# Tcadart/pyLatticeDSO

Measured on AMD Instinct MI355X. Metric: beams/s assembly+PCG-solve, higher is better.
Workload: dtype f64

## Files before the change

include/pylattice_hip.h:

```cpp
#ifndef PYLATTICE_HIP_H
#define PYLATTICE_HIP_H

#include <stdint.h>

#ifdef __cplusplus
extern "C" {
#endif

typedef struct pl_context *pl_handle;

typedef enum {
  PL_OK = 0,
  PL_ERR_ARG = -1,
  PL_ERR_HIP = -2,
  PL_ERR_STATE = -3,
  PL_ERR_NOCONV = -4,
  PL_ERR_NAN = -5,
  PL_ERR_NODEVICE = -6
} pl_status;

typedef struct {
  int64_t n_nodes;
  int64_t n_beams;
  const double *node_xyz;
// ... 185 lines not shown
                     const int32_t *beam_conn , int32_t nb,
                     const int32_t *boundary_nodes ,
                     const double *node_xyz , const double *beam_radius ,
                     const double *seg_len , const int32_t *seg_nsub ,
                     const double *u_b ,
                     const double *lam_b ,
                     double *u_full ,
                     double *lam_full ,
                     double *sens ,
                     int32_t *info );

int pl_get_records(pl_handle h, double *rec);

int pl_debug_partition(pl_handle h, int32_t *tile_of_node, int32_t *agg_of_node, int32_t *local_agg_of_node,
                       uint8_t *eliminated);

int pl_time_kernel(pl_handle h, int which, int reps, double *avg_ms);
int pl_algorithmic_bytes(pl_handle h, double *out3);
int pl_node_words_info(pl_handle h, int *classes_on, int *n_classes, int *bytes_on, int *byte_exp);
int pl_forget_history(pl_handle h);

int pl_debug_spd_solve(int device, int32_t n, const double *A, const double *b, double *x, double *quad,
                       int32_t fp32_factor);

int pl_dist_unique_id_bytes(void);
int pl_dist_unique_id(void *id_out);
int pl_dist_loopback_id(void *id_out);
int pl_dist_abort(pl_handle h);
int pl_dist_init(pl_handle h, int rank, int world, const void *unique_id, const int32_t *shared_local,
                 const int32_t *shared_global, int32_t n_shared, int32_t n_shared_global);

typedef struct pl_lattice pl_lattice;
typedef struct {
  int64_t n_nodes, n_beams, n_cell_beam, n_cell_node, n_created;
} pl_lattice_info_t;
int pl_generate_lattice(int64_t n_cells, const double *cell_coord, const double *cell_size, const double *cell_radii,
                        int32_t n_geom, int32_t n_tmpl, const double *tmpl, const int32_t *tmpl_type,
                        pl_lattice **out, pl_lattice_info_t *info);
int pl_lattice_fetch(const pl_lattice *L, double *node_xyz, int32_t *beam_conn, double *beam_radius, int32_t *beam_type,
                     int32_t *beam_cell0, int64_t *cell_beam_ptr , int64_t *cell_beam_idx,
                     int64_t *cell_node_ptr , int64_t *cell_node_idx, int32_t *created_nodes,
                     int32_t *created_beam);
void pl_lattice_free(pl_lattice *L);

int pl_penalize(int64_t n_beams, const double *node_xyz, const int32_t *beam_conn, const double *lzone ,
                double mesh_size, double *seg_len , int32_t *seg_nsub , double *pen_xyz );
// ... 16 lines not shown
```

pylatticedso_amd/_capi.py:

```python
from __future__ import annotations

import ctypes as C
import os

import numpy as np

from .timing import timing as _timing

_HERE = os.path.dirname(os.path.abspath(__file__))
LIB_PATH = os.environ.get("PYLATTICE_HIP_LIB") or os.path.join(_HERE, "libpylattice_hip.so")

PL_OK, PL_ERR_ARG, PL_ERR_HIP, PL_ERR_STATE, PL_ERR_NOCONV, PL_ERR_NAN, PL_ERR_NODEVICE = 0, -1, -2, -3, -4, -5, -6

EXPORTS = ["pl_default_opts", "pl_opts_size", "pl_stats_size", "pl_abi_version", "pl_last_error", "pl_version", "pl_lzone", "pl_create", "pl_create_ddm",
           "pl_ddm_set_preconditioner", "pl_ddm_set_geometry", "pl_ddm_update_matrices", "pl_destroy", "pl_set_bc", "pl_set_periodic",
           "pl_update_radii", "pl_set_multiplicity", "pl_update_segments", "pl_assemble", "pl_assemble_bsr", "pl_get_bsr", "pl_spmv",
           "pl_spmv_free", "pl_spmv_bsr", "pl_solve", "pl_reactions", "pl_sens", "pl_sens_gram", "pl_energy", "pl_node_mod", "pl_schur",
           "pl_stress", "pl_stress_pnorm", "pl_buckling", "pl_buckling_pnorm",
           "pl_spmv_multi", "pl_solve_multi", "pl_schur_block", "pl_geom_spmv_multi", "pl_buckling_modes", "pl_buckling_modes_sens",
           "pl_set_mass", "pl_mass_spmv_multi", "pl_vibration_modes", "pl_vibration_modes_sens",
           "pl_dyn_spmv_multi", "pl_transient",
           "pl_schur_cells", "pl_cells_recover", "pl_get_records", "pl_debug_partition", "pl_time_kernel", "pl_algorithmic_bytes", "pl_node_words_info", "pl_forget_history", "pl_debug_spd_solve", "pl_dist_unique_id_bytes",
           "pl_dist_unique_id", "pl_dist_loopback_id", "pl_dist_abort", "pl_dist_init", "pl_dist_set_peers", "pl_generate_lattice", "pl_lattice_fetch",
           "pl_lattice_free", "pl_penalize", "pl_boundary_index", "pl_boundary_index_rows"]


class PlMesh(C.Structure):
    _fields_ = [("n_nodes", C.c_int64), ("n_beams", C.c_int64), ("node_xyz", C.c_void_p),
                ("beam_conn", C.c_void_p), ("beam_radius", C.c_void_p), ("seg_len", C.c_void_p),
                ("seg_nsub", C.c_void_p)]


class PlOpts(C.Structure):
    _fields_ = [("struct_size", C.c_uint32), ("abi_version", C.c_uint32),
                ("young", C.c_double), ("poisson", C.c_double), ("kappa", C.c_double), ("pen_coef", C.c_double),
                ("device", C.c_int32), ("spmv_kernel", C.c_int32), ("precond", C.c_int32), ("reorder", C.c_int32),
                ("check_every", C.c_int32), ("lanes_per_node", C.c_int32),
                ("tile_nodes", C.c_int32), ("coarse_max_dofs", C.c_int32), ("palette", C.c_int32),
                ("local_max_dofs", C.c_int32), ("precision", C.c_int32), ("restart_every", C.c_int32),
                ("alpha_max", C.c_double), ("grid_lo", C.c_double * 3), ("grid_hi", C.c_double * 3),
                ("grid_nodes", C.c_int64), ("mintol", C.c_double), ("compact_records", C.c_int32),
                ("condense", C.c_int32), ("chol_persistent", C.c_int32), ("cg_form", C.c_int32),
                ("tile_modes", C.c_int32), ("coarse_modes", C.c_int32), ("overlap", C.c_int32),
                ("coarse_storage", C.c_int32), ("warm_start", C.c_int32), ("short_iteration", C.c_int32)]

# ... 35 lines not shown
    lib.pl_lattice_free.restype = None
    V, I32, I64, D = C.c_void_p, C.c_int32, C.c_int64, C.c_double
    sig = {"pl_default_opts": [V, C.c_uint32], "pl_opts_size": [], "pl_stats_size": [], "pl_abi_version": [], "pl_lzone": [I32, I64, I64, V, V, V, V], "pl_create": [V, V, V], "pl_create_ddm": [I64, I64, I32, V, I32, V, V, V, V],
           "pl_ddm_set_preconditioner": [V, I32, V, V], "pl_ddm_set_geometry": [V, V], "pl_ddm_update_matrices": [V, I32, V, V], "pl_destroy": [V], "pl_set_bc": [V, V, V, V], "pl_set_periodic": [V, V],
           "pl_update_radii": [V, V], "pl_set_multiplicity": [V, V], "pl_update_segments": [V, V, V], "pl_assemble": [V],
           "pl_assemble_bsr": [V, I32, V, V], "pl_get_bsr": [V, V, V, V], "pl_spmv": [V, V, V],
           "pl_spmv_free": [V, V, V], "pl_spmv_bsr": [V, V, V], "pl_solve": [V, D, I32, V, V],
           "pl_reactions": [V, V, V], "pl_sens": [V, V, V, V], "pl_sens_gram": [V, I32, V, V], "pl_energy": [V, V, V], "pl_node_mod": [V, V, V],
           "pl_stress": [V, V, I32, V, V], "pl_stress_pnorm": [V, V, I32, D, V, V, V, V],
           "pl_buckling": [V, V, I32, D, I32, V, V, V], "pl_buckling_pnorm": [V, V, I32, D, I32, D, V, V, V, V],
           "pl_schur": [V, V, I32, D, I32, V], "pl_spmv_multi": [V, I32, I32, V, V],
           "pl_solve_multi": [V, I32, V, V, D, I32, V, V], "pl_schur_block": [V, V, I32, D, I32, I32, V],
           "pl_geom_spmv_multi": [V, V, I32, I32, V, V],
           "pl_buckling_modes": [V, V, I32, I32, D, I32, D, I32, V, V, V, V, V],
           "pl_buckling_modes_sens": [V, V, I32, V, V, D, I32, V, V, V, V],
           "pl_set_mass": [V, D, I32, V], "pl_mass_spmv_multi": [V, I32, I32, V, V],
           "pl_vibration_modes": [V, I32, I32, D, I32, D, I32, V, V, V, V, V],
           "pl_vibration_modes_sens": [V, I32, V, V, V, V, V],
           "pl_dyn_spmv_multi": [V, D, D, I32, I32, V, V],
           "pl_transient": [V, I32, D, D, D, D, D, I32, V, V, V, V, D, I32, I32, V, V, V, I32, V, V, V],
           "pl_schur_cells": [V, I32, I32, I32, V, I32, V, V, V, V, V, V, V],
           "pl_cells_recover": [V, I32, I32, I32, V, I32, V, V, V, V, V, V, V, V, V, V, V],
           "pl_get_records": [V, V], "pl_debug_partition": [V, V, V, V, V], "pl_time_kernel": [V, I32, I32, V],
           "pl_algorithmic_bytes": [V, V], "pl_node_words_info": [V, V, V, V, V], "pl_forget_history": [V], "pl_debug_spd_solve": [I32, I32, V, V, V, V, I32], "pl_dist_unique_id_bytes": [], "pl_dist_unique_id": [V], "pl_dist_loopback_id": [V], "pl_dist_abort": [V],
           "pl_dist_init": [V, I32, I32, V, V, V, I32, I32], "pl_dist_set_peers": [V, V],
           "pl_generate_lattice": [I64, V, V, V, I32, I32, V, V, V, V], "pl_lattice_fetch": [V] * 12,
           "pl_lattice_free": [V], "pl_penalize": [I64, V, V, V, D, V, V, V],
           "pl_boundary_index": [I64, V, V, I64, V, V, V, V, V, V],
           "pl_boundary_index_rows": [I64, V, V, I64, V, V, V, V, V, V]}
    for name, args in sig.items():
        getattr(lib, name).argtypes = args
    if lib.pl_opts_size() != C.sizeof(PlOpts) or lib.pl_stats_size() != C.sizeof(PlStats):
        raise ImportError(f"{p}: pl_opts_t / pl_stats_t are {lib.pl_opts_size()} / {lib.pl_stats_size()} bytes in the "
                          f"library, {C.sizeof(PlOpts)} / {C.sizeof(PlStats)} in this binding (ABI version "
                          f"{lib.pl_abi_version()}): rebuild libpylattice_hip.so")
    _lib = lib
    return lib


def default_opts(lib=None) -> "PlOpts":
    lib = lib or load_library()
    opts = PlOpts()
    _check(lib, lib.pl_default_opts(C.byref(opts), C.sizeof(PlOpts)))
    return opts


def _ptr(a):
# ... 11 lines not shown
    if rc != PL_OK and rc not in allow:
        raise PlError(rc, lib.pl_last_error().decode())
    return rc


def lzone(node_xyz, beam_conn, beam_radius, device=0):
    lib = load_library()
    xyz = _f64(np.asarray(node_xyz).reshape(-1))
    conn = np.ascontiguousarray(beam_conn, dtype=np.int32).reshape(-1)
    rad = _f64(np.asarray(beam_radius).reshape(-1), len(conn) // 2)
    out = np.empty(len(conn), np.float64)
    _check(lib, lib.pl_lzone(int(device), len(xyz) // 3, len(conn) // 2, _ptr(xyz), _ptr(conn), _ptr(rad), _ptr(out)))
    return out.reshape(-1, 2)


def debug_spd_solve(A, b, device=0, fp32_factor=False):
    lib = load_library()
    A = np.ascontiguousarray(A, np.float64)
    b = np.ascontiguousarray(b, np.float64)
    x = np.empty_like(b)
    q = C.c_double()
    _check(lib, lib.pl_debug_spd_solve(device, len(b), _ptr(A), _ptr(b), _ptr(x), C.byref(q), int(bool(fp32_factor))))
    return x, q.value


MULTI_MAX = 64
SENS_GRAM_MAX = 8

SCHUR_CELLS_MAX_BOUNDARY, SCHUR_CELLS_MAX_INTERIOR, SCHUR_CELLS_MAX_BEAMS = 32, 16, 512


def schur_cells_fits(n_nodes, n_beams, n_boundary):
    return (0 < n_boundary <= SCHUR_CELLS_MAX_BOUNDARY and n_nodes - n_boundary <= SCHUR_CELLS_MAX_INTERIOR
            and 0 < n_beams <= SCHUR_CELLS_MAX_BEAMS)


def _per_instance(name, a, tail, n_inst):
    if a.shape == tail:
        a = np.broadcast_to(a, (n_inst,) + tail)
    elif a.shape != (n_inst,) + tail:
        raise ValueError(f"{name} must have shape {tail} or {(n_inst,) + tail}, got {a.shape}")
    return np.ascontiguousarray(a)


def schur_cells(node_xyz, beam_conn, boundary_nodes, beam_radius, seg_len, seg_nsub, young, poisson, kappa=0.9,
                pen_coef=1.5, device=0, n_inst=None):
# ... 755 lines not shown
```

pylatticedso_amd/csrc/pl_api.hip:

```cpp
#include <functional>

#include "pl_solver.h"
#include "pl_condense.h"
#include "pl_multi.h"
#include "pl_stress.h"
#include "pl_buckling.h"
#include "pl_geom.h"
#include "pl_mass.h"
#include "pl_dyn.h"
#include "pl_sensgram.h"


namespace {
template <typename WT>
int debug_spd_solve_t(int device, int32_t n, const double *A, const double *b, double *x, double *quad) {
  if (n <= 0 || !A || !b || !x) return fail(PL_ERR_ARG, "pl_debug_spd_solve: bad argument");
  int ndev = 0;
  if (hipGetDeviceCount(&ndev) != hipSuccess || ndev <= 0) return fail(PL_ERR_NODEVICE, "no HIP device visible");
  PL_HIP(hipSetDevice(device));
  const int np = (n + pl::kNB - 1) / pl::kNB * pl::kNB;
  std::vector<double> Ap((size_t)np * np, 0.0), bp(np, 0.0);
  for (int i = 0; i < np; ++i) {
    if (i < n) {
      std::memcpy(&Ap[(size_t)i * np], A + (size_t)i * n, n * sizeof(double));
// ... 15 lines not shown
  PL_HIP(dt.alloc(np));
  PL_HIP(dy.alloc(np));
  PL_HIP(dq.alloc(pl::kSlots));
  PL_HIP(dinfo.alloc(2));
  PL_HIP(hipMemcpy(dA.p, Ap.data(), Ap.size() * sizeof(double), hipMemcpyHostToDevice));
  PL_HIP(hipMemcpy(db.p, bp.data(), np * sizeof(double), hipMemcpyHostToDevice));
  PL_HIP(hipMemset(dW.p, 0, Ap.size() * sizeof(WT)));
  PL_HIP(hipMemset(dq.p, 0, pl::kSlots * sizeof(double)));
  PL_HIP(hipMemset(dinfo.p, 0, 2 * sizeof(int)));
  pl::dense_factor_inverse(dA.p, dL.p, dW.p, dWt.p, dD.p, np, np, dinfo.p, 0, nullptr);
  pl::dense_apply(dW.p, dWt.p, np, np, db.p, dt.p, dy.p, dq.p, nullptr, nullptr);
  PL_HIP(hipGetLastError());
  PL_HIP(hipDeviceSynchronize());
  int info[2];
  PL_HIP(hipMemcpy(info, dinfo.p, sizeof(info), hipMemcpyDeviceToHost));
  if (info[0] != 0) return fail(PL_ERR_ARG, "pl_debug_spd_solve: matrix is not positive definite");
  std::vector<double> y(np), q(pl::kSlots);
  PL_HIP(hipMemcpy(y.data(), dy.p, np * sizeof(double), hipMemcpyDeviceToHost));
  PL_HIP(hipMemcpy(q.data(), dq.p, pl::kSlots * sizeof(double), hipMemcpyDeviceToHost));
  std::memcpy(x, y.data(), n * sizeof(double));
  if (quad) {
    *quad = 0.0;
    for (double v : q) *quad += v;
  }
  return PL_OK;
}

}

extern "C" {

const char *pl_last_error(void) { return g_err.c_str(); }
#ifndef PL_KP_HASH
#define PL_KP_HASH "unknown"
#endif
const char *pl_version(void) { return "pylattice_hip 0.2 (gfx950) kp=" PL_KP_HASH; }

uint32_t pl_opts_size(void) { return (uint32_t)sizeof(pl_opts_t); }
uint32_t pl_stats_size(void) { return (uint32_t)sizeof(pl_stats_t); }
uint32_t pl_abi_version(void) { return PL_ABI_VERSION; }

int pl_default_opts(pl_opts_t *o, uint32_t struct_size) {
  if (!o) return fail(PL_ERR_ARG, "pl_default_opts: null argument");
  if (struct_size != sizeof(pl_opts_t))
    return fail(PL_ERR_ARG, "pl_default_opts: the caller's pl_opts_t has " + std::to_string(struct_size) +
                                " bytes, this library's " + std::to_string(sizeof(pl_opts_t)) +
// ... 2873 lines not shown
  PL_HIP(hipEventElapsedTime(&ms, h->ev0, h->ev1));
  *avg_ms = (double)ms / reps;
  return PL_OK;
}

int pl_node_words_info(pl_handle h, int *classes_on, int *n_classes, int *bytes_on, int *byte_exp) {
  if (!valid(h)) return fail(PL_ERR_ARG, "pl_node_words_info: null handle");
  const pl::Coarse &cs = h->coarse;
  const bool words = node_words_apply(h);
  const bool cls = words && h->assembled && cs.dcl_ready;
  const bool bytes = words && cs.rel_e >= 0;
  if (classes_on) *classes_on = cls ? 1 : 0;
  if (n_classes) *n_classes = h->assembled ? cs.dcl_classes : 0;
  if (bytes_on) *bytes_on = bytes ? 1 : 0;
  if (byte_exp) *byte_exp = bytes ? cs.rel_e : -1;
  return PL_OK;
}

int pl_debug_spd_solve(int device, int32_t n, const double *A, const double *b, double *x, double *quad,
                       int32_t fp32_factor) {
  return fp32_factor ? debug_spd_solve_t<float>(device, n, A, b, x, quad)
                     : debug_spd_solve_t<double>(device, n, A, b, x, quad);
}

int pl_lzone(int device, int64_t n_nodes, int64_t n_beams, const double *node_xyz, const int32_t *beam_conn,
             const double *beam_radius, double *lzone) {
  if (n_nodes <= 0 || n_beams <= 0 || !node_xyz || !beam_conn || !beam_radius || !lzone)
    return fail(PL_ERR_ARG, "pl_lzone: bad argument");
  int ndev = 0;
  if (hipGetDeviceCount(&ndev) != hipSuccess || ndev <= 0)
    return fail(PL_ERR_NODEVICE, "pl_lzone: no HIP device visible (libpylattice_hip has no CPU fallback)");
  if (device < 0 || device >= ndev) return fail(PL_ERR_ARG, "pl_lzone: bad device ordinal");
  const int64_t nh = 2 * n_beams;
  std::vector<int64_t> ptr((size_t)n_nodes + 1, 0);
  for (int64_t h = 0; h < nh; ++h) {
    const int32_t v = beam_conn[h];
    if (v < 0 || v >= n_nodes) return fail(PL_ERR_ARG, "pl_lzone: node id out of range");
    ptr[(size_t)v + 1]++;
  }
  for (int64_t i = 0; i < n_nodes; ++i) ptr[i + 1] += ptr[i];
  std::vector<int32_t> half((size_t)nh);
  {
    std::vector<int64_t> fill(ptr.begin(), ptr.end() - 1);
    for (int64_t h = 0; h < nh; ++h) half[(size_t)fill[beam_conn[h]]++] = (int32_t)h;
  }
  PL_HIP(hipSetDevice(device));
// ... 117 lines not shown
```

pylatticedso_amd/csrc/pl_dense.h:

```cpp
#pragma once
#include <hip/hip_runtime.h>

#include <functional>

#include <algorithm>

#include "pl_kernels.h"

namespace pl {

constexpr int kNB = 64;
constexpr int kLdT = kNB + 2;

__device__ __forceinline__ void tile_fma(const double *At, const double *Bt, int tx, int ty, double acc[4][4]) {
#pragma unroll 8
  for (int k = 0; k < kNB; ++k) {
    double a[4], b[4];
#pragma unroll
    for (int q = 0; q < 4; ++q) {
      a[q] = At[k * kLdT + 4 * ty + q];
      b[q] = Bt[k * kLdT + 4 * tx + q];
    }
#pragma unroll
    for (int i = 0; i < 4; ++i)
#pragma unroll
      for (int j = 0; j < 4; ++j) acc[i][j] += a[i] * b[j];
  }
}

__device__ __forceinline__ void stage_rows_as_k_minor(const double *G, int ld, double *T) {
  for (int e = threadIdx.x; e < kNB * kNB; e += kBlock) {
    const int row = e / kNB, k = e % kNB;
    T[k * kLdT + row] = G[(size_t)row * ld + k];
  }
}
__device__ __forceinline__ void stage_rows_as_k_major(const double *G, int ld, double *T) {
  for (int e = threadIdx.x; e < kNB * kNB; e += kBlock) {
    const int k = e / kNB, col = e % kNB;
    T[k * kLdT + col] = G[(size_t)k * ld + col];
  }
}

__device__ __forceinline__ void tile_fetch(const double *__restrict__ G, int ld, double regs[kNB * kNB / kBlock]) {
#pragma unroll
  for (int q = 0; q < kNB * kNB / kBlock; ++q) {
    const int e = threadIdx.x + q * kBlock;
    regs[q] = G[(size_t)(e / kNB) * ld + e % kNB];
  }
}
__device__ __forceinline__ void tile_store_k_minor(const double regs[kNB * kNB / kBlock], double *T) {
#pragma unroll
  for (int q = 0; q < kNB * kNB / kBlock; ++q) {
    const int e = threadIdx.x + q * kBlock;
    T[(e % kNB) * kLdT + e / kNB] = regs[q];
  }
}

constexpr int kLdD = kNB + 1;
constexpr int kHalf = kNB / 2;

constexpr int kDiagLds = kNB * kLdD + kHalf * (kHalf + 1) + kNB * 4 + 16 + 2;

__device__ __forceinline__ void chol_diag_body(double a[4][4], double *__restrict__ Akk, int ld, int kb,
                                               double *__restrict__ Dinv, int *__restrict__ info, double *lds) {
  double *Ls = lds, *T = Ls + kNB * kLdD, *colt = T + kHalf * (kHalf + 1), *dm = colt + kNB * 4;
  int &bad_s = *reinterpret_cast<int *>(dm + 16);
  static_assert(kNB == 64 && kBlock == 256, "chol_diag_body is written for 64 x 64 blocks and 256 threads");
  const int tx = threadIdx.x & 15, ty = threadIdx.x >> 4;
  const bool act = ty >= tx;
  if (threadIdx.x == 0) bad_s = 0;
  __syncthreads();
  for (int jt = 0; jt < kNB / 4; ++jt) {
    if (tx == jt && ty == jt) {
      double l[4][4], m[4][4];
      bool ok = true;
#pragma unroll
      for (int c = 0; c < 4; ++c) {
        double d = a[c][c];
#pragma unroll
        for (int q = 0; q < c; ++q) d -= l[c][q] * l[c][q];
        ok = ok && (d > 0.0);
        const double ri = rsqrt(d > 0.0 ? d : 1.0);
        l[c][c] = (d > 0.0 ? d : 1.0) * ri;
        m[c][c] = ri;
#pragma unroll
        for (int i = c + 1; i < 4; ++i) {
          double v = a[i][c];
#pragma unroll
          for (int q = 0; q < c; ++q) v -= l[i][q] * l[c][q];
          l[i][c] = v * ri;
        }
      }
      if (!ok) bad_s = 1;
#pragma unroll
      for (int c = 0; c < 4; ++c)
#pragma unroll
        for (int i = c + 1; i < 4; ++i) {
          double v = 0.0;
#pragma unroll
          for (int q = c; q < i; ++q) v -= l[i][q] * m[q][c];
          m[i][c] = v * m[i][i];
        }
#pragma unroll
      for (int i = 0; i < 4; ++i)
#pragma unroll
        for (int c = 0; c < 4; ++c) {
          a[i][c] = c <= i ? l[i][c] : 0.0;
          dm[4 * i + c] = c <= i ? m[i][c] : 0.0;
        }
    }
    __syncthreads();
    if (tx == jt && ty > jt) {
      double mm[16];
#pragma unroll
      for (int e = 0; e < 16; ++e) mm[e] = dm[e];
      double l[4][4];
#pragma unroll
      for (int i = 0; i < 4; ++i)
#pragma unroll
        for (int c = 0; c < 4; ++c) {
          double v = 0.0;
#pragma unroll
          for (int q = 0; q <= c; ++q) v += a[i][q] * mm[4 * c + q];
          l[i][c] = v;
        }
#pragma unroll
      for (int i = 0; i < 4; ++i)
#pragma unroll
        for (int c = 0; c < 4; ++c) {
          a[i][c] = l[i][c];
          colt[(4 * ty + i) * 4 + c] = l[i][c];
        }
    }
    __syncthreads();
    if (act && tx > jt) {
      double rv[4][4], cv[4][4];
#pragma unroll
      for (int i = 0; i < 4; ++i)
#pragma unroll
        for (int q = 0; q < 4; ++q) {
          rv[i][q] = colt[(4 * ty + i) * 4 + q];
          cv[i][q] = colt[(4 * tx + i) * 4 + q];
        }
#pragma unroll
      for (int i = 0; i < 4; ++i)
#pragma unroll
        for (int c = 0; c < 4; ++c)
#pragma unroll
          for (int q = 0; q < 4; ++q) a[i][c] -= rv[i][q] * cv[c][q];
    }
  }
#pragma unroll
  for (int i = 0; i < 4; ++i)
#pragma unroll
    for (int c = 0; c < 4; ++c) {
      const int row = 4 * ty + i, cx = 4 * tx + c;
      const double v = (act && cx <= row) ? a[i][c] : 0.0;
      Ls[row * kLdD + cx] = v;
      Akk[(size_t)row * ld + cx] = v;
    }
  __syncthreads();
  if (bad_s && threadIdx.x == 0) info[0] = kb * kNB + 1;
  const int lane = threadIdx.x & 63, wv = threadIdx.x >> 6;
  if (wv < 2 && lane < kHalf) {
    const int o = kHalf * wv;
    double x[kHalf];
#pragma unroll
    for (int i = 0; i < kHalf; ++i) {
      double sacc = (lane == i) ? 1.0 : 0.0;
#pragma unroll
      for (int m = 0; m < i; ++m) sacc -= Ls[(o + i) * kLdD + o + m] * x[m];
      x[i] = sacc / Ls[(o + i) * kLdD + o + i];
    }
#pragma unroll
    for (int i = 0; i < kHalf; ++i) Ls[(o + i) * kLdD + o + lane] = x[i];
  }
  __syncthreads();
  const int r = threadIdx.x & (kHalf - 1), cg = threadIdx.x / kHalf;
  {
    double t4[4] = {0, 0, 0, 0};
#pragma unroll 8
    for (int m = 0; m < kHalf; ++m) {
      const double l = Ls[(kHalf + r) * kLdD + m];
#pragma unroll
      for (int q = 0; q < 4; ++q) t4[q] += l * Ls[m * kLdD + 4 * cg + q];
    }
#pragma unroll
    for (int q = 0; q < 4; ++q) T[r * (kHalf + 1) + 4 * cg + q] = t4[q];
  }
  __syncthreads();
  {
    double o4[4] = {0, 0, 0, 0};
#pragma unroll 8
    for (int m = 0; m < kHalf; ++m) {
      const double xv = Ls[(kHalf + r) * kLdD + kHalf + m];
#pragma unroll
      for (int q = 0; q < 4; ++q) o4[q] += xv * T[m * (kHalf + 1) + 4 * cg + q];
    }
#pragma unroll
    for (int q = 0; q < 4; ++q) Ls[(kHalf + r) * kLdD + 4 * cg + q] = -o4[q];
  }
  __syncthreads();
  double *Dk = Dinv + (size_t)kb * kNB * kNB;
  for (int e = threadIdx.x; e < kNB * kNB; e += kBlock) Dk[e] = Ls[(e / kNB) * kLdD + e % kNB];
}

__global__ __launch_bounds__(kBlock) void k_chol_diag(double *__restrict__ A, int ld, int kb,
                                                     double *__restrict__ Dinv, int *__restrict__ info) {
  __shared__ double lds[kDiagLds];
  const int tx = threadIdx.x & 15, ty = threadIdx.x >> 4;
  double *Akk = A + ((size_t)kb * kNB) * ld + (size_t)kb * kNB;
  double a[4][4];
#pragma unroll
  for (int i = 0; i < 4; ++i)
#pragma unroll
    for (int c = 0; c < 4; ++c) a[i][c] = ty >= tx ? Akk[(size_t)(4 * ty + i) * ld + 4 * tx + c] : 0.0;
  chol_diag_body(a, Akk, ld, kb, Dinv, info, lds);
}

__device__ __forceinline__ void chol_step_body(double *__restrict__ A, double *__restrict__ Lf, int ld, int kb, int ib,
                                               int jb, double *__restrict__ Dinv, int *__restrict__ info, double *S) {
  double *X = S, *Y = S + kNB * kLdT, *D = S + 2 * kNB * kLdT;
  static_assert(kDiagLds <= 2 * kNB * kLdT, "diagonal-block scratch must fit into X|Y");
  const int tx = threadIdx.x & 15, ty = threadIdx.x >> 4;
  double *Aij = A + ((size_t)ib * kNB) * ld + (size_t)jb * kNB;
  double rd[kNB * kNB / kBlock], rj[kNB * kNB / kBlock], ri[kNB * kNB / kBlock], a[4][4];
  tile_fetch(Dinv + (size_t)kb * kNB * kNB, kNB, rd);
  tile_fetch(A + ((size_t)jb * kNB) * ld + (size_t)kb * kNB, ld, rj);
  if (ib != jb) tile_fetch(A + ((size_t)ib * kNB) * ld + (size_t)kb * kNB, ld, ri);
#pragma unroll
  for (int i = 0; i < 4; ++i)
#pragma unroll
    for (int j = 0; j < 4; ++j) a[i][j] = Aij[(size_t)(4 * ty + i) * ld + 4 * tx + j];
  tile_store_k_minor(rd, D);
  tile_store_k_minor(rj, X);
  __syncthreads();
  {
    double l[4][4] = {};
    tile_fma(X, D, tx, ty, l);
#pragma unroll
    for (int i = 0; i < 4; ++i)
#pragma unroll
      for (int j = 0; j < 4; ++j) Y[(4 * tx + j) * kLdT + 4 * ty + i] = l[i][j];
    if (ib == jb) {
      double *Lg = Lf + ((size_t)ib * kNB) * ld + (size_t)kb * kNB;
#pragma unroll
      for (int i = 0; i < 4; ++i)
#pragma unroll
        for (int j = 0; j < 4; ++j) Lg[(size_t)(4 * ty + i) * ld + 4 * tx + j] = l[i][j];
    }
  }
  __syncthreads();
  const double *Li = Y;
  if (ib != jb) {
    tile_store_k_minor(ri, X);
    __syncthreads();
    double l[4][4] = {};
    tile_fma(X, D, tx, ty, l);
    __syncthreads();
#pragma unroll
    for (int i = 0; i < 4; ++i)
#pragma unroll
      for (int j = 0; j < 4; ++j) X[(4 * tx + j) * kLdT + 4 * ty + i] = l[i][j];
    __syncthreads();
    Li = X;
  }
  double acc[4][4] = {};
  tile_fma(Li, Y, tx, ty, acc);
#pragma unroll
  for (int i = 0; i < 4; ++i)
#pragma unroll
    for (int j = 0; j < 4; ++j) a[i][j] -= acc[i][j];
  if (ib == kb + 1 && jb == kb + 1) {
    __syncthreads();
#pragma unroll
    for (int i = 0; i < 4; ++i)
#pragma unroll
      for (int j = 0; j < 4; ++j)
        if (ty < tx) a[i][j] = 0.0;
    chol_diag_body(a, Aij, ld, kb + 1, Dinv, info, X);
    return;
  }
#pragma unroll
  for (int i = 0; i < 4; ++i)
#pragma unroll
    for (int j = 0; j < 4; ++j) Aij[(size_t)(4 * ty + i) * ld + 4 * tx + j] = a[i][j];
}

__global__ __launch_bounds__(kBlock) void k_chol_step(double *__restrict__ A, double *__restrict__ Lf, int ld, int kb,
                                                      double *__restrict__ Dinv, int *__restrict__ info) {
  __shared__ double S[3 * kNB * kLdT];
  const int ib = kb + 1 + blockIdx.x, jb = kb + 1 + blockIdx.y;
  if (jb > ib) return;
  chol_step_body(A, Lf, ld, kb, ib, jb, Dinv, info, S);
}

constexpr int kChainMaxGrid = 196;
__device__ __forceinline__ bool chain_barrier(unsigned *bar, unsigned target, int *info) {
  __syncthreads();
  __shared__ int ok;
  if (threadIdx.x == 0) {
    __threadfence();
    atomicAdd(bar, 1u);
    int good = 1;
    unsigned spins = 0;
    while (__hip_atomic_load(bar, __ATOMIC_RELAXED, __HIP_MEMORY_SCOPE_AGENT) < target) {
      __builtin_amdgcn_s_sleep(1);
      if (++spins > (1u << 26) || __hip_atomic_load(info, __ATOMIC_RELAXED, __HIP_MEMORY_SCOPE_AGENT) == -7) {
        atomicExch(info, -7);
// ... 90 lines not shown
      o0 += a * S[m * kCw + 2 * g];
      o1 += a * S[m * kCw + 2 * g + 1];
    }
    WT *Wik = W + ((size_t)ib * kNB + r) * ld + (size_t)kb * kNB + c0 + 2 * g;
    Wik[0] = (WT)(-o0);
    Wik[1] = (WT)(-o1);
    WT *Wtki = Wt + ((size_t)kb * kNB + c0 + 2 * g) * ld + (size_t)ib * kNB + r;
    Wtki[0] = (WT)(-o0);
    Wtki[ld] = (WT)(-o1);
    if (RING && scratch && row1 < nb && ib + bw >= row1) {
      double *sc = scratch + ((size_t)kb * kNB + c0 + 2 * g) * ld + (size_t)ib * kNB + r;
      sc[0] = -o0;
      sc[ld] = -o1;
    }
    if (RING) {
      double *slot = Ws + (ib % kRing) * kNB * kCw;
      slot[r * kCw + 2 * g] = -o0;
      slot[r * kCw + 2 * g + 1] = -o1;
    }
  }
}

constexpr int kCwM = 16;
typedef double v4f64 __attribute__((ext_vector_type(4)));
template <typename WT>
__global__ __launch_bounds__(kBlock) void k_trtri_cols_mfma(const double *__restrict__ L, int ld, int nb, int bw,
                                                            const double *__restrict__ Dinv, WT *__restrict__ W,
                                                            WT *__restrict__ Wt, int row0 = 0, int row1 = 1 << 30) {
  __shared__ double At[kNB * kLdT];
  __shared__ double Ws[kNB * kCwM], S[kNB * kCwM];
  constexpr int kSl = kNB / kCwM;
  constexpr int kWr = kNB * kCwM / kBlock;
  const int kb = blockIdx.x / kSl, c0 = (blockIdx.x % kSl) * kCwM;
  row1 = min(row1, nb);
  if (kb >= row1) return;
  const bool first = kb >= row0;
  const int lane = threadIdx.x & 63, wv = threadIdx.x >> 6;
  const int li = lane & 15, lk = lane >> 4;
  if (first)
    for (int e = threadIdx.x; e < kNB * kCwM; e += kBlock) {
      const int row = e / kCwM, c = e % kCwM;
      const double v = Dinv[(size_t)kb * kNB * kNB + (size_t)row * kNB + c0 + c];
      W[((size_t)kb * kNB + row) * ld + (size_t)kb * kNB + c0 + c] = (WT)v;
      Wt[((size_t)kb * kNB + c0 + c) * ld + (size_t)kb * kNB + row] = (WT)v;
    }
  const int ib0 = first ? kb + 1 : row0;
  auto slice_fetch = [&](int jb, WT wr[kWr]) {
// ... 249 lines not shown
```

pylatticedso_amd/csrc/pl_small.h:

```cpp
#pragma once
#include "pl_coarse.h"

namespace pl {

typedef double v4f64_small __attribute__((ext_vector_type(4)));

__device__ __forceinline__ double w_entry(const float *W, size_t i) { return (double)W[i]; }
__device__ __forceinline__ double w_entry(const bf16_t *W, size_t i) {
  return (double)__uint_as_float((unsigned)reinterpret_cast<const uint16_t *>(W)[i] << 16);
}

template <typename WT>
__global__ __launch_bounds__(256) void k_dense_explicit_inverse(int n, const WT *__restrict__ W, int ld,
                                                                float *__restrict__ Ainv) {
  const int lane = threadIdx.x & 63, i = lane & 15, kq = lane >> 4;
  const int nt = n / 32;
  const long q = (long)blockIdx.x * 4 + (threadIdx.x >> 6);
  if (q >= (long)nt * (nt + 1) / 2) return;
  int ti = (int)((sqrt(8.0 * (double)q + 1.0) - 1.0) * 0.5);
  while ((long)(ti + 1) * (ti + 2) / 2 <= q) ++ti;
  while ((long)ti * (ti + 1) / 2 > q) --ti;
  const int tj = (int)(q - (long)ti * (ti + 1) / 2);
  const int a0 = 32 * ti, b0 = 32 * tj;
  v4f64_small acc[2][2];
#pragma unroll
  for (int u = 0; u < 2; ++u)
#pragma unroll
    for (int v = 0; v < 2; ++v) acc[u][v] = v4f64_small{0.0, 0.0, 0.0, 0.0};
  for (int k0 = a0; k0 < n; k0 += 8) {
    double A[2][2], B[2][2];
#pragma unroll
    for (int h = 0; h < 2; ++h) {
      const size_t row = (size_t)(k0 + 4 * h + kq) * ld;
      A[h][0] = w_entry(W, row + a0 + i);
      A[h][1] = w_entry(W, row + a0 + 16 + i);
      B[h][0] = w_entry(W, row + b0 + i);
      B[h][1] = w_entry(W, row + b0 + 16 + i);
    }
#pragma unroll
    for (int h = 0; h < 2; ++h)
#pragma unroll
      for (int u = 0; u < 2; ++u)
#pragma unroll
        for (int v = 0; v < 2; ++v) acc[u][v] = __builtin_amdgcn_mfma_f64_16x16x4f64(A[h][u], B[h][v], acc[u][v], 0, 0, 0);
  }
#pragma unroll
  for (int u = 0; u < 2; ++u)
#pragma unroll
    for (int v = 0; v < 2; ++v)
#pragma unroll
      for (int r = 0; r < 4; ++r) {
        const int a = a0 + 16 * u + kq + 4 * r, b = b0 + 16 * v + i;
        const float val = (float)acc[u][v][r];
        if (ti != tj) {
          Ainv[(size_t)a * ld + b] = val;
          Ainv[(size_t)b * ld + a] = val;
        } else if (b <= a) {
          Ainv[(size_t)a * ld + b] = val;
          Ainv[(size_t)b * ld + a] = val;
        }
      }
}

template <int TM>
__global__ __launch_bounds__(kBlock) void k_small_z(const int32_t *__restrict__ tile_start,
                                                    const int32_t *__restrict__ agg_of_tile, const double *__restrict__ cen,
                                                    const double *__restrict__ xyz, const double *__restrict__ r,
// ... 98 lines not shown
```

Baseline: 253.0 million.

## Use f64 MFMA in dense Cholesky step and simplify diagonal block inverse

Replaces the scalar 4x4 FMA tile product in the blocked Cholesky update with f64 16x16x4 MFMA instructions. The diagonal-block inverse is now built during the per-column factor sweep instead of by a separate triangular solve and product afterwards. The explicit-inverse kernel gains software prefetching of several k-steps of W. A debug entry point for the factorization is also added. The coarse/local dense factor is likely only a small part of assembly plus PCG, so the effect on the metric may be limited, and the inverse rework risks numerical or correctness regressions.

```diff
diff --git a/include/pylattice_hip.h b/include/pylattice_hip.h
--- a/include/pylattice_hip.h
+++ b/include/pylattice_hip.h
@@ -231,6 +231,8 @@
 
 int pl_debug_spd_solve(int device, int32_t n, const double *A, const double *b, double *x, double *quad,
                        int32_t fp32_factor);
+int pl_debug_spd_factor(int device, int32_t n, const double *A, int32_t bw_blocks, int32_t trtri_rows, double *L_out,
+                        double *W_out, float *Ainv32_out, int32_t *info_out);
 
 int pl_dist_unique_id_bytes(void);
 int pl_dist_unique_id(void *id_out);
diff --git a/pylatticedso_amd/_capi.py b/pylatticedso_amd/_capi.py
--- a/pylatticedso_amd/_capi.py
+++ b/pylatticedso_amd/_capi.py
@@ -20,7 +20,7 @@
            "pl_spmv_multi", "pl_solve_multi", "pl_schur_block", "pl_geom_spmv_multi", "pl_buckling_modes", "pl_buckling_modes_sens",
            "pl_set_mass", "pl_mass_spmv_multi", "pl_vibration_modes", "pl_vibration_modes_sens",
            "pl_dyn_spmv_multi", "pl_transient",
-           "pl_schur_cells", "pl_cells_recover", "pl_get_records", "pl_debug_partition", "pl_time_kernel", "pl_algorithmic_bytes", "pl_node_words_info", "pl_forget_history", "pl_debug_spd_solve", "pl_dist_unique_id_bytes",
+           "pl_schur_cells", "pl_cells_recover", "pl_get_records", "pl_debug_partition", "pl_time_kernel", "pl_algorithmic_bytes", "pl_node_words_info", "pl_forget_history", "pl_debug_spd_solve", "pl_debug_spd_factor", "pl_dist_unique_id_bytes",
            "pl_dist_unique_id", "pl_dist_loopback_id", "pl_dist_abort", "pl_dist_init", "pl_dist_set_peers", "pl_generate_lattice", "pl_lattice_fetch",
            "pl_lattice_free", "pl_penalize", "pl_boundary_index", "pl_boundary_index_rows"]
 
@@ -102,7 +102,7 @@
            "pl_schur_cells": [V, I32, I32, I32, V, I32, V, V, V, V, V, V, V],
            "pl_cells_recover": [V, I32, I32, I32, V, I32, V, V, V, V, V, V, V, V, V, V, V],
            "pl_get_records": [V, V], "pl_debug_partition": [V, V, V, V, V], "pl_time_kernel": [V, I32, I32, V],
-           "pl_algorithmic_bytes": [V, V], "pl_node_words_info": [V, V, V, V, V], "pl_forget_history": [V], "pl_debug_spd_solve": [I32, I32, V, V, V, V, I32], "pl_dist_unique_id_bytes": [], "pl_dist_unique_id": [V], "pl_dist_loopback_id": [V], "pl_dist_abort": [V],
+           "pl_algorithmic_bytes": [V, V], "pl_node_words_info": [V, V, V, V, V], "pl_forget_history": [V], "pl_debug_spd_solve": [I32, I32, V, V, V, V, I32], "pl_debug_spd_factor": [I32, I32, V, I32, I32, V, V, V, V], "pl_dist_unique_id_bytes": [], "pl_dist_unique_id": [V], "pl_dist_loopback_id": [V], "pl_dist_abort": [V],
            "pl_dist_init": [V, I32, I32, V, V, V, I32, I32], "pl_dist_set_peers": [V, V],
            "pl_generate_lattice": [I64, V, V, V, I32, I32, V, V, V, V], "pl_lattice_fetch": [V] * 12,
            "pl_lattice_free": [V], "pl_penalize": [I64, V, V, V, D, V, V, V],
@@ -160,6 +160,20 @@
     q = C.c_double()
     _check(lib, lib.pl_debug_spd_solve(device, len(b), _ptr(A), _ptr(b), _ptr(x), C.byref(q), int(bool(fp32_factor))))
     return x, q.value
+
+
+def debug_spd_factor(A, bw_blocks=0, trtri_rows=0, explicit_inverse=False, device=0):
+    lib = load_library()
+    A = np.ascontiguousarray(A, np.float64)
+    n = A.shape[0]
+    npad = (n + 63) // 64 * 64
+    L = np.empty((npad, npad), np.float64)
+    W = np.empty((npad, npad), np.float64)
+    Ainv = np.empty((npad, npad), np.float32) if explicit_inverse else None
+    info = np.zeros(1, np.int32)
+    _check(lib, lib.pl_debug_spd_factor(device, n, _ptr(A), int(bw_blocks), int(trtri_rows), _ptr(L), _ptr(W), _ptr(Ainv),
+                                        _ptr(info)))
+    return L, W, Ainv, int(info[0])
 
 
 MULTI_MAX = 64
diff --git a/pylatticedso_amd/csrc/pl_api.hip b/pylatticedso_amd/csrc/pl_api.hip
--- a/pylatticedso_amd/csrc/pl_api.hip
+++ b/pylatticedso_amd/csrc/pl_api.hip
@@ -61,6 +61,87 @@
   if (quad) {
     *quad = 0.0;
     for (double v : q) *quad += v;
+  }
+  return PL_OK;
+}
+
+int debug_spd_factor(int device, int32_t n, const double *A, int32_t bw_blocks, int32_t trtri_rows, double *L_out,
+                     double *W_out, float *Ainv32_out, int32_t *info_out) {
+  if (n <= 0 || !A || !L_out || !W_out || !info_out || bw_blocks < 0 || trtri_rows < 0)
+    return fail(PL_ERR_ARG, "pl_debug_spd_factor: bad argument");
+  int ndev = 0;
+  if (hipGetDeviceCount(&ndev) != hipSuccess || ndev <= 0) return fail(PL_ERR_NODEVICE, "no HIP device visible");
+  PL_HIP(hipSetDevice(device));
+  const int np = (n + pl::kNB - 1) / pl::kNB * pl::kNB, nb = np / pl::kNB;
+  const size_t nn = (size_t)np * np;
+  std::vector<double> Ap(nn, 0.0), Lh(nn), Wh(nn);
+  for (int i = 0; i < np; ++i) {
+    if (i < n) std::memcpy(&Ap[(size_t)i * np], A + (size_t)i * n, n * sizeof(double));
+    else Ap[(size_t)i * np + i] = 1.0;
+  }
+  DevBuf<double> dA, dL, dD, dW, dWt;
+  DevBuf<float> dW32, dAinv;
+  DevBuf<int> dinfo;
+  PL_HIP(dA.alloc(nn));
+  PL_HIP(dL.alloc(nn));
+  PL_HIP(dW.alloc(nn));
+  PL_HIP(dWt.alloc(nn));
+  PL_HIP(dD.alloc((size_t)np * pl::kNB));
+  PL_HIP(dinfo.alloc(2));
+  PL_HIP(hipMemcpy(dA.p, Ap.data(), nn * sizeof(double), hipMemcpyHostToDevice));
+  PL_HIP(hipMemset(dL.p, 0, nn * sizeof(double)));
+  PL_HIP(hipMemset(dW.p, 0, nn * sizeof(double)));
+  PL_HIP(hipMemset(dWt.p, 0, nn * sizeof(double)));
+  PL_HIP(hipMemset(dinfo.p, 0, 2 * sizeof(int)));
+  struct Side {
+    hipStream_t s = nullptr, s2 = nullptr;
+    hipEvent_t e0 = nullptr, e1 = nullptr;
+    ~Side() {
+      if (e0) (void)hipEventDestroy(e0);
+      if (e1) (void)hipEventDestroy(e1);
+      if (s2) (void)hipStreamDestroy(s2);
+      if (s) (void)hipStreamDestroy(s);
+    }
+  } sd;
+  PL_HIP(hipStreamCreateWithFlags(&sd.s, hipStreamNonBlocking));
+  pl::TrtriPhases ph;
+  if (trtri_rows > 0) {
+    PL_HIP(hipStreamCreateWithFlags(&sd.s2, hipStreamNonBlocking));
+    PL_HIP(hipEventCreateWithFlags(&sd.e0, hipEventDisableTiming));
+    PL_HIP(hipEventCreateWithFlags(&sd.e1, hipEventDisableTiming));
+    ph.stream = sd.s2;
+    ph.ev_go = sd.e0;
+    ph.ev_done = sd.e1;
+    ph.rows = trtri_rows;
+  }
+  pl::dense_factor_inverse(dA.p, dL.p, dW.p, dWt.p, dD.p, np, np, dinfo.p, bw_blocks, sd.s, nullptr, nullptr, ph);
+  PL_HIP(hipGetLastError());
+  PL_HIP(hipStreamSynchronize(sd.s));
+  int info[2];
+  PL_HIP(hipMemcpy(info, dinfo.p, sizeof(info), hipMemcpyDeviceToHost));
+  info_out[0] = info[0];
+  PL_HIP(hipMemcpy(Ap.data(), dA.p, nn * sizeof(double), hipMemcpyDeviceToHost));
+  PL_HIP(hipMemcpy(Lh.data(), dL.p, nn * sizeof(double), hipMemcpyDeviceToHost));
+  PL_HIP(hipMemcpy(Wh.data(), dW.p, nn * sizeof(double), hipMemcpyDeviceToHost));
+  for (int kb = 0; kb < nb; ++kb)
+    for (int r = 0; r < pl::kNB; ++r)
+      std::memcpy(&Lh[((size_t)kb * pl::kNB + r) * np + (size_t)kb * pl::kNB],
+                  &Ap[((size_t)kb * pl::kNB + r) * np + (size_t)kb * pl::kNB], pl::kNB * sizeof(double));
+  std::memcpy(L_out, Lh.data(), nn * sizeof(double));
+  std::memcpy(W_out, Wh.data(), nn * sizeof(double));
+  if (Ainv32_out) {
+    std::vector<float> W32(nn);
+    for (size_t e = 0; e < nn; ++e) W32[e] = (float)Wh[e];
+    PL_HIP(dW32.alloc(nn));
+    PL_HIP(dAinv.alloc(nn));
+    PL_HIP(hipMemcpy(dW32.p, W32.data(), nn * sizeof(float), hipMemcpyHostToDevice));
+    PL_HIP(hipMemset(dAinv.p, 0, nn * sizeof(float)));
+    const long tiles = (long)(np / 32) * (np / 32 + 1) / 2;
+    hipLaunchKernelGGL(pl::k_dense_explicit_inverse<float>, dim3((unsigned)((tiles + 3) / 4)), dim3(256), 0, sd.s, np,
+                       (const float *)dW32.p, np, dAinv.p);
+    PL_HIP(hipGetLastError());
+    PL_HIP(hipStreamSynchronize(sd.s));
+    PL_HIP(hipMemcpy(Ainv32_out, dAinv.p, nn * sizeof(float), hipMemcpyDeviceToHost));
   }
   return PL_OK;
 }
@@ -2980,6 +3061,10 @@
   return fp32_factor ? debug_spd_solve_t<float>(device, n, A, b, x, quad)
                      : debug_spd_solve_t<double>(device, n, A, b, x, quad);
 }
+int pl_debug_spd_factor(int device, int32_t n, const double *A, int32_t bw_blocks, int32_t trtri_rows, double *L_out,
+                        double *W_out, float *Ainv32_out, int32_t *info_out) {
+  return debug_spd_factor(device, n, A, bw_blocks, trtri_rows, L_out, W_out, Ainv32_out, info_out);
+}
 
 int pl_lzone(int device, int64_t n_nodes, int64_t n_beams, const double *node_xyz, const int32_t *beam_conn,
              const double *beam_radius, double *lzone) {
diff --git a/pylatticedso_amd/csrc/pl_dense.h b/pylatticedso_amd/csrc/pl_dense.h
--- a/pylatticedso_amd/csrc/pl_dense.h
+++ b/pylatticedso_amd/csrc/pl_dense.h
@@ -12,19 +12,16 @@
 constexpr int kNB = 64;
 constexpr int kLdT = kNB + 2;
 
-__device__ __forceinline__ void tile_fma(const double *At, const double *Bt, int tx, int ty, double acc[4][4]) {
-#pragma unroll 8
-  for (int k = 0; k < kNB; ++k) {
-    double a[4], b[4];
-#pragma unroll
-    for (int q = 0; q < 4; ++q) {
-      a[q] = At[k * kLdT + 4 * ty + q];
-      b[q] = Bt[k * kLdT + 4 * tx + q];
-    }
-#pragma unroll
-    for (int i = 0; i < 4; ++i)
-#pragma unroll
-      for (int j = 0; j < 4; ++j) acc[i][j] += a[i] * b[j];
+typedef double v4f64 __attribute__((ext_vector_type(4)));
+__device__ __forceinline__ void tile_mfma(const double *At, const double *Bt, int wv, int li, int lk, v4f64 acc[4]) {
+#pragma unroll
+  for (int s4 = 0; s4 < kNB / 4; ++s4) {
+    const double a = At[(4 * s4 + lk) * kLdT + 16 * wv + li];
+#pragma unroll
+    for (int cb = 0; cb < 4; ++cb) {
+      const double b = Bt[(4 * s4 + lk) * kLdT + 16 * cb + li];
+      acc[cb] = __builtin_amdgcn_mfma_f64_16x16x4f64(a, b, acc[cb], 0, 0, 0);
+    }
   }
 }
 
@@ -56,18 +53,16 @@
   }
 }
 
-constexpr int kLdD = kNB + 1;
-constexpr int kHalf = kNB / 2;
-
-constexpr int kDiagLds = kNB * kLdD + kHalf * (kHalf + 1) + kNB * 4 + 16 + 2;
+constexpr int kDiagLds = 2 * kNB * 4 + 16 + 2;
 
 __device__ __forceinline__ void chol_diag_body(double a[4][4], double *__restrict__ Akk, int ld, int kb,
                                                double *__restrict__ Dinv, int *__restrict__ info, double *lds) {
-  double *Ls = lds, *T = Ls + kNB * kLdD, *colt = T + kHalf * (kHalf + 1), *dm = colt + kNB * 4;
+  double *colt = lds, *xrow = colt + kNB * 4, *dm = xrow + kNB * 4;
   int &bad_s = *reinterpret_cast<int *>(dm + 16);
   static_assert(kNB == 64 && kBlock == 256, "chol_diag_body is written for 64 x 64 blocks and 256 threads");
   const int tx = threadIdx.x & 15, ty = threadIdx.x >> 4;
   const bool act = ty >= tx;
+  double mj[4][4];
   if (threadIdx.x == 0) bad_s = 0;
   __syncthreads();
   for (int jt = 0; jt < kNB / 4; ++jt) {
@@ -79,9 +74,10 @@
         double d = a[c][c];
 #pragma unroll
         for (int q = 0; q < c; ++q) d -= l[c][q] * l[c][q];
-        ok = ok && (d > 0.0);
-        const double ri = rsqrt(d > 0.0 ? d : 1.0);
-        l[c][c] = (d > 0.0 ? d : 1.0) * ri;
+        const bool pos = d > 0.0;
+        ok = ok && pos;
+        const double ri = pos ? rsqrt(d) : 0.0;
+        l[c][c] = pos ? d * ri : 1.0;
         m[c][c] = ri;
 #pragma unroll
         for (int i = c + 1; i < 4; ++i) {
@@ -106,11 +102,13 @@
 #pragma unroll
         for (int c = 0; c < 4; ++c) {
           a[i][c] = c <= i ? l[i][c] : 0.0;
-          dm[4 * i + c] = c <= i ? m[i][c] : 0.0;
+          mj[i][c] = c <= i ? m[i][c] : 0.0;
+          dm[4 * i + c] = mj[i][c];
+          xrow[16 * jt + 4 * c + i] = mj[i][c];
         }
     }
     __syncthreads();
-    if (tx == jt && ty > jt) {
+    if (tx == jt && ty != jt) {
       double mm[16];
 #pragma unroll
       for (int e = 0; e < 16; ++e) mm[e] = dm[e];
@@ -124,23 +122,25 @@
           for (int q = 0; q <= c; ++q) v += a[i][q] * mm[4 * c + q];
           l[i][c] = v;
         }
+      double *pub = (ty > jt ? colt : xrow) + 16 * ty;
 #pragma unroll
       for (int i = 0; i < 4; ++i)
 #pragma unroll
         for (int c = 0; c < 4; ++c) {
           a[i][c] = l[i][c];
-          colt[(4 * ty + i) * 4 + c] = l[i][c];
+          pub[4 * i + c] = l[i][c];
         }
     }
     __syncthreads();
-    if (act && tx > jt) {
+    if (tx > jt && (act || ty <= jt)) {
+      const double *ps = (act ? colt : xrow) + 16 * ty, *qs = colt + 16 * tx;
       double rv[4][4], cv[4][4];
 #pragma unroll
       for (int i = 0; i < 4; ++i)
 #pragma unroll
         for (int q = 0; q < 4; ++q) {
-          rv[i][q] = colt[(4 * ty + i) * 4 + q];
-          cv[i][q] = colt[(4 * tx + i) * 4 + q];
+          rv[i][q] = ps[4 * i + q];
+          cv[i][q] = qs[4 * i + q];
         }
 #pragma unroll
       for (int i = 0; i < 4; ++i)
@@ -150,59 +150,21 @@
           for (int q = 0; q < 4; ++q) a[i][c] -= rv[i][q] * cv[c][q];
     }
   }
+  if (bad_s && threadIdx.x == 0) info[0] = kb * kNB + 1;
+  double *Dk = Dinv + (size_t)kb * kNB * kNB;
 #pragma unroll
   for (int i = 0; i < 4; ++i)
 #pragma unroll
     for (int c = 0; c < 4; ++c) {
-      const int row = 4 * ty + i, cx = 4 * tx + c;
-      const double v = (act && cx <= row) ? a[i][c] : 0.0;
-      Ls[row * kLdD + cx] = v;
-      Akk[(size_t)row * ld + cx] = v;
-    }
-  __syncthreads();
-  if (bad_s && threadIdx.x == 0) info[0] = kb * kNB + 1;
-  const int lane = threadIdx.x & 63, wv = threadIdx.x >> 6;
-  if (wv < 2 && lane < kHalf) {
-    const int o = kHalf * wv;
-    double x[kHalf];
-#pragma unroll
-    for (int i = 0; i < kHalf; ++i) {
-      double sacc = (lane == i) ? 1.0 : 0.0;
-#pragma unroll
-      for (int m = 0; m < i; ++m) sacc -= Ls[(o + i) * kLdD + o + m] * x[m];
-      x[i] = sacc / Ls[(o + i) * kLdD + o + i];
-    }
-#pragma unroll
-    for (int i = 0; i < kHalf; ++i) Ls[(o + i) * kLdD + o + lane] = x[i];
-  }
-  __syncthreads();
-  const int r = threadIdx.x & (kHalf - 1), cg = threadIdx.x / kHalf;
-  {
-    double t4[4] = {0, 0, 0, 0};
-#pragma unroll 8
-    for (int m = 0; m < kHalf; ++m) {
-      const double l = Ls[(kHalf + r) * kLdD + m];
-#pragma unroll
-      for (int q = 0; q < 4; ++q) t4[q] += l * Ls[m * kLdD + 4 * cg + q];
-    }
-#pragma unroll
-    for (int q = 0; q < 4; ++q) T[r * (kHalf + 1) + 4 * cg + q] = t4[q];
-  }
-  __syncthreads();
-  {
-    double o4[4] = {0, 0, 0, 0};
-#pragma unroll 8
-    for (int m = 0; m < kHalf; ++m) {
-      const double xv = Ls[(kHalf + r) * kLdD + kHalf + m];
-#pragma unroll
-      for (int q = 0; q < 4; ++q) o4[q] += xv * T[m * (kHalf + 1) + 4 * cg + q];
-    }
-#pragma unroll
-    for (int q = 0; q < 4; ++q) Ls[(kHalf + r) * kLdD + 4 * cg + q] = -o4[q];
-  }
-  __syncthreads();
-  double *Dk = Dinv + (size_t)kb * kNB * kNB;
-  for (int e = threadIdx.x; e < kNB * kNB; e += kBlock) Dk[e] = Ls[(e / kNB) * kLdD + e % kNB];
+      if (act) {
+        Akk[(size_t)(4 * ty + i) * ld + 4 * tx + c] = a[i][c];
+        if (ty == tx) Dk[(4 * ty + i) * kNB + 4 * tx + c] = mj[i][c];
+      } else {
+        Akk[(size_t)(4 * ty + i) * ld + 4 * tx + c] = 0.0;
+        Dk[(4 * ty + i) * kNB + 4 * tx + c] = 0.0;
+        Dk[(4 * tx + i) * kNB + 4 * ty + c] = a[c][i];
+      }
+    }
 }
 
 __global__ __launch_bounds__(kBlock) void k_chol_diag(double *__restrict__ A, int ld, int kb,
@@ -221,33 +183,34 @@
 __device__ __forceinline__ void chol_step_body(double *__restrict__ A, double *__restrict__ Lf, int ld, int kb, int ib,
                                                int jb, double *__restrict__ Dinv, int *__restrict__ info, double *S) {
   double *X = S, *Y = S + kNB * kLdT, *D = S + 2 * kNB * kLdT;
-  static_assert(kDiagLds <= 2 * kNB * kLdT, "diagonal-block scratch must fit into X|Y");
-  const int tx = threadIdx.x & 15, ty = threadIdx.x >> 4;
+  static_assert(kDiagLds <= kNB * kLdT, "diagonal-block scratch must fit into Y");
+  const int lane = threadIdx.x & 63, wv = threadIdx.x >> 6, li = lane & 15, lk = lane >> 4;
   double *Aij = A + ((size_t)ib * kNB) * ld + (size_t)jb * kNB;
-  double rd[kNB * kNB / kBlock], rj[kNB * kNB / kBlock], ri[kNB * kNB / kBlock], a[4][4];
+  double rd[kNB * kNB / kBlock], rj[kNB * kNB / kBlock], ri[kNB * kNB / kBlock];
+  v4f64 a[4];
   tile_fetch(Dinv + (size_t)kb * kNB * kNB, kNB, rd);
   tile_fetch(A + ((size_t)jb * kNB) * ld + (size_t)kb * kNB, ld, rj);
   if (ib != jb) tile_fetch(A + ((size_t)ib * kNB) * ld + (size_t)kb * kNB, ld, ri);
 #pragma unroll
-  for (int i = 0; i < 4; ++i)
-#pragma unroll
-    for (int j = 0; j < 4; ++j) a[i][j] = Aij[(size_t)(4 * ty + i) * ld + 4 * tx + j];
+  for (int cb = 0; cb < 4; ++cb)
+#pragma unroll
+    for (int q = 0; q < 4; ++q) a[cb][q] = Aij[(size_t)(16 * wv + lk + 4 * q) * ld + 16 * cb + li];
   tile_store_k_minor(rd, D);
   tile_store_k_minor(rj, X);
   __syncthreads();
   {
-    double l[4][4] = {};
-    tile_fma(X, D, tx, ty, l);
-#pragma unroll
-    for (int i = 0; i < 4; ++i)
-#pragma unroll
-      for (int j = 0; j < 4; ++j) Y[(4 * tx + j) * kLdT + 4 * ty + i] = l[i][j];
+    v4f64 l[4] = {};
+    tile_mfma(X, D, wv, li, lk, l);
+#pragma unroll
+    for (int cb = 0; cb < 4; ++cb)
+#pragma unroll
+      for (int q = 0; q < 4; ++q) Y[(16 * cb + li) * kLdT + 16 * wv + lk + 4 * q] = l[cb][q];
     if (ib == jb) {
       double *Lg = Lf + ((size_t)ib * kNB) * ld + (size_t)kb * kNB;
 #pragma unroll
-      for (int i = 0; i < 4; ++i)
-#pragma unroll
-        for (int j = 0; j < 4; ++j) Lg[(size_t)(4 * ty + i) * ld + 4 * tx + j] = l[i][j];
+      for (int cb = 0; cb < 4; ++cb)
+#pragma unroll
+        for (int q = 0; q < 4; ++q) Lg[(size_t)(16 * wv + lk + 4 * q) * ld + 16 * cb + li] = l[cb][q];
     }
   }
   __syncthreads();
@@ -255,36 +218,40 @@
   if (ib != jb) {
     tile_store_k_minor(ri, X);
     __syncthreads();
-    double l[4][4] = {};
-    tile_fma(X, D, tx, ty, l);
-    __syncthreads();
+    v4f64 l[4] = {};
+    tile_mfma(X, D, wv, li, lk, l);
+    __syncthreads();
+#pragma unroll
+    for (int cb = 0; cb < 4; ++cb)
+#pragma unroll
+      for (int q = 0; q < 4; ++q) X[(16 * cb + li) * kLdT + 16 * wv + lk + 4 * q] = l[cb][q];
+    __syncthreads();
+    Li = X;
+  }
+  v4f64 acc[4] = {};
+  tile_mfma(Li, Y, wv, li, lk, acc);
+#pragma unroll
+  for (int cb = 0; cb < 4; ++cb) a[cb] -= acc[cb];
+  if (ib == kb + 1 && jb == kb + 1) {
+    __syncthreads();
+#pragma unroll
+    for (int cb = 0; cb < 4; ++cb)
+#pragma unroll
+      for (int q = 0; q < 4; ++q) X[(16 * wv + lk + 4 * q) * kLdT + 16 * cb + li] = a[cb][q];
+    __syncthreads();
+    const int tx = threadIdx.x & 15, ty = threadIdx.x >> 4;
+    double t[4][4];
 #pragma unroll
     for (int i = 0; i < 4; ++i)
 #pragma unroll
-      for (int j = 0; j < 4; ++j) X[(4 * tx + j) * kLdT + 4 * ty + i] = l[i][j];
-    __syncthreads();
-    Li = X;
-  }
-  double acc[4][4] = {};
-  tile_fma(Li, Y, tx, ty, acc);
-#pragma unroll
-  for (int i = 0; i < 4; ++i)
-#pragma unroll
-    for (int j = 0; j < 4; ++j) a[i][j] -= acc[i][j];
-  if (ib == kb + 1 && jb == kb + 1) {
-    __syncthreads();
-#pragma unroll
-    for (int i = 0; i < 4; ++i)
-#pragma unroll
-      for (int j = 0; j < 4; ++j)
-        if (ty < tx) a[i][j] = 0.0;
-    chol_diag_body(a, Aij, ld, kb + 1, Dinv, info, X);
+      for (int j = 0; j < 4; ++j) t[i][j] = ty >= tx ? X[(4 * ty + i) * kLdT + 4 * tx + j] : 0.0;
+    chol_diag_body(t, Aij, ld, kb + 1, Dinv, info, Y);
     return;
   }
 #pragma unroll
-  for (int i = 0; i < 4; ++i)
-#pragma unroll
-    for (int j = 0; j < 4; ++j) Aij[(size_t)(4 * ty + i) * ld + 4 * tx + j] = a[i][j];
+  for (int cb = 0; cb < 4; ++cb)
+#pragma unroll
+    for (int q = 0; q < 4; ++q) Aij[(size_t)(16 * wv + lk + 4 * q) * ld + 16 * cb + li] = a[cb][q];
 }
 
 __global__ __launch_bounds__(kBlock) void k_chol_step(double *__restrict__ A, double *__restrict__ Lf, int ld, int kb,
@@ -421,7 +388,6 @@
 }
 
 constexpr int kCwM = 16;
-typedef double v4f64 __attribute__((ext_vector_type(4)));
 template <typename WT>
 __global__ __launch_bounds__(kBlock) void k_trtri_cols_mfma(const double *__restrict__ L, int ld, int nb, int bw,
                                                             const double *__restrict__ Dinv, WT *__restrict__ W,
diff --git a/pylatticedso_amd/csrc/pl_small.h b/pylatticedso_amd/csrc/pl_small.h
--- a/pylatticedso_amd/csrc/pl_small.h
+++ b/pylatticedso_amd/csrc/pl_small.h
@@ -4,11 +4,6 @@
 namespace pl {
 
 typedef double v4f64_small __attribute__((ext_vector_type(4)));
-
-__device__ __forceinline__ double w_entry(const float *W, size_t i) { return (double)W[i]; }
-__device__ __forceinline__ double w_entry(const bf16_t *W, size_t i) {
-  return (double)__uint_as_float((unsigned)reinterpret_cast<const uint16_t *>(W)[i] << 16);
-}
 
 template <typename WT>
 __global__ __launch_bounds__(256) void k_dense_explicit_inverse(int n, const WT *__restrict__ W, int ld,
@@ -27,22 +22,42 @@
   for (int u = 0; u < 2; ++u)
 #pragma unroll
     for (int v = 0; v < 2; ++v) acc[u][v] = v4f64_small{0.0, 0.0, 0.0, 0.0};
-  for (int k0 = a0; k0 < n; k0 += 8) {
-    double A[2][2], B[2][2];
+  constexpr int kEiTrips = 4;
+  WT cur[kEiTrips][2][4], nxt[kEiTrips][2][4];
+  auto fetch = [&](int k0, WT dst[kEiTrips][2][4]) {
 #pragma unroll
-    for (int h = 0; h < 2; ++h) {
-      const size_t row = (size_t)(k0 + 4 * h + kq) * ld;
-      A[h][0] = w_entry(W, row + a0 + i);
-      A[h][1] = w_entry(W, row + a0 + 16 + i);
-      B[h][0] = w_entry(W, row + b0 + i);
-      B[h][1] = w_entry(W, row + b0 + 16 + i);
+    for (int t = 0; t < kEiTrips; ++t)
+#pragma unroll
+      for (int h = 0; h < 2; ++h) {
+        const size_t row = (size_t)(k0 + 8 * t + 4 * h + kq) * ld;
+        dst[t][h][0] = W[row + a0 + i];
+        dst[t][h][1] = W[row + a0 + 16 + i];
+        dst[t][h][2] = W[row + b0 + i];
+        dst[t][h][3] = W[row + b0 + 16 + i];
+      }
+  };
+  fetch(a0, cur);
+  for (int k0 = a0; k0 < n; k0 += 8 * kEiTrips) {
+    const bool more = k0 + 8 * kEiTrips < n;
+    if (more) fetch(k0 + 8 * kEiTrips, nxt);
+#pragma unroll
+    for (int t = 0; t < kEiTrips; ++t)
+#pragma unroll
+      for (int h = 0; h < 2; ++h) {
+        const double A[2] = {(double)cur[t][h][0], (double)cur[t][h][1]}, B[2] = {(double)cur[t][h][2], (double)cur[t][h][3]};
+#pragma unroll
+        for (int u = 0; u < 2; ++u)
+#pragma unroll
+          for (int v = 0; v < 2; ++v) acc[u][v] = __builtin_amdgcn_mfma_f64_16x16x4f64(A[u], B[v], acc[u][v], 0, 0, 0);
+      }
+    if (more) {
+#pragma unroll
+      for (int t = 0; t < kEiTrips; ++t)
+#pragma unroll
+        for (int h = 0; h < 2; ++h)
+#pragma unroll
+          for (int e = 0; e < 4; ++e) cur[t][h][e] = nxt[t][h][e];
     }
-#pragma unroll
-    for (int h = 0; h < 2; ++h)
-#pragma unroll
-      for (int u = 0; u < 2; ++u)
-#pragma unroll
-        for (int v = 0; v < 2; ++v) acc[u][v] = __builtin_amdgcn_mfma_f64_16x16x4f64(A[h][u], B[h][v], acc[u][v], 0, 0, 0);
   }
 #pragma unroll
   for (int u = 0; u < 2; ++u)
```

New measurement: 257.4 million, median of 6. Within noise of the previous version (+1.7%).
